# zju3dv/NeuralRecon-W

Hardware: NVIDIA H100
Metric: training rays/sec (higher is better)
Workload: dtype bf16 (3-product split forward, plain bf16 backward, fp32 accumulate)

## Files before the change

### neuralrecon-w_b200/csrc/epilogue_fast.cuh

```cuda
#pragma once
#include "epilogue_tc.cuh"

namespace nrw {

enum EpiKind {
  EK_GENERIC = 0,
  EK_FWD_SOFTPLUS,
  EK_FWD_RELU,
  EK_FWD_NONE,
  EK_GATE_FWD,
  EK_TANGENT,
  EK_REVERSE,
  EK_RELU_BWD,
  EK_FWD_HEAD,
  EK_COUNT
};

inline int pick_epi_kind(const Epi& e) {
  auto al16 = [](const void* p) { return (reinterpret_cast<uintptr_t>(p) & 15) == 0; };
  auto rows16 = [&](const void* p, int ld) { return !p || (al16(p) && (ld & 3) == 0); };
  if (e.head_w || e.head_partial)
    return (e.head_w && e.head_partial && e.bias && al16(e.bias) && al16(e.head_w) && e.act == ACT_SOFTPLUS100 && e.scale == 1.0f && e.n_planes == 0 &&
            !e.atomic && !e.aux_u.p && !e.rowvec && !e.aux_relu && !e.out_pre && !e.out2 && !e.out_f32 &&
            !e.colsum && !e.aux_add && e.n_store >= (1 << 29)) ? EK_FWD_HEAD : -1;
  if (e.atomic || e.n_planes > 3) return EK_GENERIC;
  if (e.n_planes > 0 && (!al16(e.out_pl.p) || (e.out_pl.ld & 3) || (e.out_pl.pstride & 7))) return EK_GENERIC;
  if (e.aux_u.p && (!al16(e.aux_u.p) || (e.aux_u.ld & 3) || (e.aux_u.pstride & 7))) return EK_GENERIC;
  if (!rows16(e.out_pre.p, e.out_pre.ld) || !rows16(e.out2.p, e.out2.ld) || !rows16(e.aux_add.p, e.aux_add.ld) ||
      !rows16(e.aux_q.p, e.aux_q_bcast ? 0 : e.aux_q.ld) || !rows16(e.out_f32, e.ld_f32) || !rows16(e.aux_relu, e.ld_relu) ||
      !al16(e.bias) || !al16(e.colvec))
    return EK_GENERIC;
  const bool gate = e.aux_u.p != nullptr;
  if (gate && e.out_pre && !e.out2 && !e.aux_add && !e.colsum && !e.bias && !e.rowvec && !e.aux_relu && e.n_planes > 0 && !e.out_f32)
    return EK_GATE_FWD;
  if (gate && e.out2 && e.aux_q && !e.out_pre && !e.bias && !e.rowvec && !e.aux_add && !e.colsum && !e.aux_relu &&
      ((e.n_planes > 0) != (e.out_f32 != nullptr)))
    return EK_TANGENT;
  if (gate && e.aux_add && !e.out2 && !e.out_pre && !e.bias && !e.aux_relu && e.n_planes > 0 && !e.out_f32) return EK_REVERSE;
  if (!gate && e.aux_relu && !e.out_pre && !e.out2 && !e.aux_add && !e.bias && e.n_planes > 0 && !e.out_f32 && e.act == ACT_NONE)
    return EK_RELU_BWD;
  if (!gate && e.bias && !e.rowvec && !e.aux_relu && !e.aux_add && !e.out_pre && !e.out2 && !e.out_f32 && !e.colsum && e.n_planes > 0) {
    if (e.act == ACT_SOFTPLUS100) return EK_FWD_SOFTPLUS;
    if (e.act == ACT_RELU) return EK_FWD_RELU;
    if (e.act == ACT_NONE) return EK_FWD_NONE;
  }
  return EK_GENERIC;
}

#define NRW_GATE_K (-144.269504088896341f)

template <int EK>
__device__ __forceinline__ void epi_fast16(const Epi& e, float* stg, const float (&v)[16], int m0w, int nc, int M, int N, int lane,
                                           float* cs_tile, float* hacc) {
  if constexpr (EK == EK_GENERIC) {
    epi_chunk16(e, stg, v, m0w, nc, M, N, lane, cs_tile);
  } else if constexpr (EK == EK_FWD_HEAD) {
    const int col = nc + (lane & 3) * 4;
    const float4 b = ldg4(e.bias + col), hw = ldg4(e.head_w + col);
    float x[16];
    line_transpose(stg, v, lane, x);
#pragma unroll
    for (int it = 0; it < 4; ++it) {
      float p = softplus100(x[4 * it] + b.x) * hw.x;
      p = fmaf(softplus100(x[4 * it + 1] + b.y), hw.y, p);
      p = fmaf(softplus100(x[4 * it + 2] + b.z), hw.z, p);
      p = fmaf(softplus100(x[4 * it + 3] + b.w), hw.w, p);
      p += __shfl_xor_sync(0xFFFFFFFFu, p, 1);
      p += __shfl_xor_sync(0xFFFFFFFFu, p, 2);
      hacc[it] += p;
    }
  } else {
    if (M - m0w < 32 || N - nc < 16 || e.n_store - nc < 16) {
      epi_chunk16(e, stg, v, m0w, nc, M, N, lane, cs_tile);
      return;
    }
    const int col = nc + (lane & 3) * 4;
    const long long row = (long long)m0w + (lane >> 2);
    float u[16];
    float s[16];
    float4 b;
    if constexpr (EK == EK_GATE_FWD || EK == EK_TANGENT || EK == EK_REVERSE) {
      tile_load_bf16(e.aux_u.p + row * e.aux_u.ld + col, e.aux_u.ld, u);
      if constexpr (EK == EK_GATE_FWD) {
        if (e.aux_u_planes > 1) tile_load_bf16(e.aux_u.plane(1) + row * e.aux_u.ld + col, e.aux_u.ld, s);
      }
    }
    if constexpr (EK == EK_FWD_SOFTPLUS || EK == EK_FWD_RELU || EK == EK_FWD_NONE) b = ldg4(e.bias + col);
    if constexpr (EK == EK_TANGENT) {
      if (e.aux_q_bcast) {
        const float4 qb = ldg4(e.aux_q.f32() + col);
#pragma unroll
        for (int it = 0; it < 4; ++it) { s[4 * it] = qb.x; s[4 * it + 1] = qb.y; s[4 * it + 2] = qb.z; s[4 * it + 3] = qb.w; }
      } else {
        tile_load(e.aux_q, row, col, s);
      }
    }
    if constexpr (EK == EK_REVERSE) tile_load(e.aux_add, row, col, s);
    if constexpr (EK == EK_RELU_BWD) tile_load_bf16(e.aux_relu + row * e.ld_relu + col, e.ld_relu, u);
    float x[16], w[16];
    line_transpose(stg, v, lane, x);

    if constexpr (EK == EK_FWD_SOFTPLUS || EK == EK_FWD_RELU || EK == EK_FWD_NONE) {
      const float bb[4] = {b.x, b.y, b.z, b.w};
#pragma unroll
      for (int i = 0; i < 16; ++i) {
        const float t = x[i] + bb[i & 3];
        if constexpr (EK == EK_FWD_SOFTPLUS) w[i] = softplus100(t) * e.scale;
        else if constexpr (EK == EK_FWD_RELU) w[i] = fmaxf(t, 0.0f) * e.scale;
        else w[i] = t * e.scale;
      }
    }
    if constexpr (EK == EK_REVERSE || EK == EK_RELU_BWD) {
      if (e.rowvec) {
        const float4 c = ldg4(e.colvec + col);
        const float cc[4] = {c.x, c.y, c.z, c.w};
#pragma unroll
        for (int it = 0; it < 4; ++it) {
          const float rv = __ldg(e.rowvec + row + it * 8);
#pragma unroll
          for (int k = 0; k < 4; ++k) x[4 * it + k] = fmaf(rv, cc[k], x[4 * it + k]);
        }
      }
    }
    if constexpr (EK == EK_GATE_FWD) tile_store(e.out_pre, row, col, x);
    if constexpr (EK == EK_GATE_FWD || EK == EK_TANGENT || EK == EK_REVERSE) {
      if constexpr (EK == EK_GATE_FWD) {
        if (e.aux_u_planes > 1) {
#pragma unroll
          for (int i = 0; i < 16; ++i) u[i] += s[i];
        }
      }
      for (int pl = EK == EK_GATE_FWD ? 2 : 1; pl < e.aux_u_planes; ++pl) {
        float t[16];
        tile_load_bf16(e.aux_u.plane(pl) + row * e.aux_u.ld + col, e.aux_u.ld, t);
#pragma unroll
        for (int i = 0; i < 16; ++i) u[i] += t[i];
      }
      const float kk = NRW_GATE_K * e.aux_u_scale, sc = e.scale;
      if constexpr (EK == EK_TANGENT) {
        const float sc100 = 100.0f * sc;
#pragma unroll
        for (int i = 0; i < 16; ++i) {
          const float ee = mufu_ex2(u[i] * kk);
          const float s1 = 1.0f - ee;
          const float xs = x[i] * s1;
          w[i] = xs * sc;
          s[i] = (xs * s[i]) * (ee * sc100);
        }
        tile_store(e.out2, row, col, s);
      } else if constexpr (EK == EK_REVERSE) {
#pragma unroll
        for (int i = 0; i < 16; ++i) {
          const float ee = mufu_ex2(u[i] * kk);
          w[i] = fmaf(x[i], fmaf(-sc, ee, sc), s[i]);
        }
      } else {
#pragma unroll
        for (int i = 0; i < 16; ++i) {
          const float ee = mufu_ex2(u[i] * kk);
          w[i] = x[i] * fmaf(-sc, ee, sc);
        }
      }
    }
    if constexpr (EK == EK_RELU_BWD) {
#pragma unroll
      for (int i = 0; i < 16; ++i) w[i] = u[i] > 0.0f ? x[i] * e.scale : 0.0f;
    }
    if constexpr (EK == EK_REVERSE || EK == EK_RELU_BWD) {
      if (cs_tile) line_colsum_add(w, lane, cs_tile);
    }
    if constexpr (EK == EK_TANGENT) {
      if (e.out_f32) tile_store_f32(e.out_f32 + row * e.ld_f32 + col, e.ld_f32, w);
    }
    for (int pl = 0; pl < e.n_planes; ++pl) {
      uint32_t pk[8];
      if (pl + 1 < e.n_planes) split_plane<16>(w, pk);
      else pack_bf16(w, pk);
      tile_store_bf16(e.out_pl.plane(pl) + row * e.out_pl.ld + col, e.out_pl.ld, pk);
    }
  }
}

}
```

### neuralrecon-w_b200/csrc/epilogue_tc.cuh

```cuda
#pragma once
#include "epilogue.cuh"

namespace nrw {

struct LineLayout {
  int sl;
  int r0;
  int rows_valid;
  bool full;
};

__device__ __forceinline__ bool aligned16(const void* p) { return (reinterpret_cast<uintptr_t>(p) & 15) == 0; }
__device__ __forceinline__ bool aligned8(const void* p) { return (reinterpret_cast<uintptr_t>(p) & 7) == 0; }

__device__ __forceinline__ void line_transpose(float* stg, const float (&v)[16], int lane, float (&x)[16]) {
  const int sl = lane & 3, r0 = lane >> 2;
#pragma unroll
  for (int s = 0; s < 4; ++s)
    *reinterpret_cast<float4*>(stg + lane * 16 + ((s ^ ((lane >> 1) & 3)) << 2)) = make_float4(v[4 * s], v[4 * s + 1], v[4 * s + 2], v[4 * s + 3]);
  __syncwarp();
#pragma unroll
  for (int it = 0; it < 4; ++it) {
    const int rr = it * 8 + r0;
    const float4 t = *reinterpret_cast<const float4*>(stg + rr * 16 + ((sl ^ ((rr >> 1) & 3)) << 2));
    x[4 * it] = t.x; x[4 * it + 1] = t.y; x[4 * it + 2] = t.z; x[4 * it + 3] = t.w;
  }
  __syncwarp();
}

__device__ __forceinline__ float4 ldg4(const float* p) {
  float4 v;
  asm volatile("ld.global.nc.L2::256B.v4.f32 {%0, %1, %2, %3}, [%4];" : "=f"(v.x), "=f"(v.y), "=f"(v.z), "=f"(v.w) : "l"(p));
  return v;
}
__device__ __forceinline__ uint2 ldg2u(const bf16* p) {
  uint2 v;
  asm volatile("ld.global.nc.L2::256B.v2.u32 {%0, %1}, [%2];" : "=r"(v.x), "=r"(v.y) : "l"(p));
  return v;
}

__device__ __forceinline__ void tile_load_f32(const float* p, long long ld, float (&o)[16]) {
#pragma unroll
  for (int it = 0; it < 4; ++it) {
    const float4 t = ldg4(p + it * 8 * ld);
    o[4 * it] = t.x; o[4 * it + 1] = t.y; o[4 * it + 2] = t.z; o[4 * it + 3] = t.w;
  }
}
__device__ __forceinline__ void tile_load_bf16(const bf16* p, long long ld, float (&o)[16]) {
#pragma unroll
  for (int it = 0; it < 4; ++it) {
    const uint2 t = ldg2u(p + it * 8 * ld);
    o[4 * it] = __uint_as_float(t.x << 16); o[4 * it + 1] = __uint_as_float(t.x & 0xFFFF0000u);
    o[4 * it + 2] = __uint_as_float(t.y << 16); o[4 * it + 3] = __uint_as_float(t.y & 0xFFFF0000u);
  }
}
__device__ __forceinline__ void tile_store_f32(float* p, long long ld, const float (&o)[16]) {
#pragma unroll
  for (int it = 0; it < 4; ++it)
    *reinterpret_cast<float4*>(p + it * 8 * ld) = make_float4(o[4 * it], o[4 * it + 1], o[4 * it + 2], o[4 * it + 3]);
}
__device__ __forceinline__ void tile_store_bf16(bf16* p, long long ld, const uint32_t (&pk)[8]) {
#pragma unroll
  for (int it = 0; it < 4; ++it) *reinterpret_cast<uint2*>(p + it * 8 * ld) = make_uint2(pk[2 * it], pk[2 * it + 1]);
}
__device__ __forceinline__ void pack_bf16(const float (&w)[16], uint32_t (&pk)[8]) {
#pragma unroll
  for (int t = 0; t < 8; ++t) {
    const __nv_bfloat162 h = __floats2bfloat162_rn(w[2 * t], w[2 * t + 1]);
    pk[t] = *reinterpret_cast<const uint32_t*>(&h);
  }
}
__device__ __forceinline__ void tile_load(const SideStream& s, long long row, int col, float (&o)[16]) {
  if (s.is_bf16()) tile_load_bf16(s.h() + row * s.ld + col, s.ld, o);
  else tile_load_f32(s.f32() + row * s.ld + col, s.ld, o);
}
__device__ __forceinline__ void tile_store(const SideStream& s, long long row, int col, const float (&o)[16]) {
  if (s.is_bf16()) {
    uint32_t pk[8];
    pack_bf16(o, pk);
    tile_store_bf16(s.h() + row * s.ld + col, s.ld, pk);
  } else {
    tile_store_f32(s.f32() + row * s.ld + col, s.ld, o);
  }
}

__device__ __forceinline__ bool line_fast(const LineLayout& L, const void* p, long long ld, int ncols) {
  return L.full && ncols >= 16 && aligned16(p) && (ld & 3) == 0;
}
__device__ __forceinline__ void line_load_f32(const LineLayout& L, const float* __restrict__ src, long long ld, int ncols,
                                              float (&o)[16]) {
  if (line_fast(L, src, ld, ncols)) {
    tile_load_f32(src + L.r0 * ld + L.sl * 4, ld, o);
    return;
  }
#pragma unroll
  for (int it = 0; it < 4; ++it) {
    const int rr = it * 8 + L.r0;
#pragma unroll
    for (int k = 0; k < 4; ++k) {
      const int c = L.sl * 4 + k;
      o[4 * it + k] = (rr < L.rows_valid && c < ncols) ? src[(long long)rr * ld + c] : 0.0f;
    }
  }
}
__device__ __forceinline__ void line_store_f32(const LineLayout& L, float* __restrict__ dst, long long ld, int ncols,
                                               const float (&o)[16], bool atomic) {
  if (!atomic && line_fast(L, dst, ld, ncols)) {
    tile_store_f32(dst + L.r0 * ld + L.sl * 4, ld, o);
    return;
  }
#pragma unroll
  for (int it = 0; it < 4; ++it) {
    const int rr = it * 8 + L.r0;
#pragma unroll
    for (int k = 0; k < 4; ++k) {
      const int c = L.sl * 4 + k;
      if (rr < L.rows_valid && c < ncols) {
        if (atomic) atomicAdd(dst + (long long)rr * ld + c, o[4 * it + k]);
        else dst[(long long)rr * ld + c] = o[4 * it + k];
      }
    }
  }
}
__device__ __forceinline__ void line_store_bf16(const LineLayout& L, bf16* __restrict__ dst, long long ld, int ncols,
                                                const uint32_t (&pk)[8]) {
  if (L.full && ncols >= 16 && aligned8(dst) && (ld & 3) == 0) {
    tile_store_bf16(dst + L.r0 * ld + L.sl * 4, ld, pk);
    return;
  }
#pragma unroll
  for (int it = 0; it < 4; ++it) {
    const int rr = it * 8 + L.r0;
#pragma unroll
    for (int k = 0; k < 4; ++k) {
      const int c = L.sl * 4 + k;
      if (rr < L.rows_valid && c < ncols)
        dst[(long long)rr * ld + c] = __ushort_as_bfloat16((unsigned short)((pk[2 * it + (k >> 1)] >> ((k & 1) * 16)) & 0xFFFFu));
    }
  }
}
__device__ __forceinline__ void line_load_planes(const LineLayout& L, const Planes& P, int n_planes, long long m0w, int nc, int ncols,
                                                 float scale, float (&o)[16]) {
#pragma unroll
  for (int i = 0; i < 16; ++i) o[i] = 0.0f;
  for (int pl = 0; pl < n_planes; ++pl) {
    const bf16* src = P.plane(pl) + m0w * P.ld + nc;
    if (L.full && ncols >= 16 && aligned8(src) && (P.ld & 3) == 0) {
      float t[16];
      tile_load_bf16(src + L.r0 * P.ld + L.sl * 4, P.ld, t);
#pragma unroll
      for (int i = 0; i < 16; ++i) o[i] += t[i];
    } else {
#pragma unroll
      for (int it = 0; it < 4; ++it) {
        const int rr = it * 8 + L.r0;
#pragma unroll
        for (int k = 0; k < 4; ++k) {
          const int c = L.sl * 4 + k;
          if (rr < L.rows_valid && c < ncols) o[4 * it + k] += __bfloat162float(src[(long long)rr * P.ld + c]);
        }
      }
    }
  }
  if (scale != 1.0f) {
#pragma unroll
    for (int i = 0; i < 16; ++i) o[i] *= scale;
  }
}
__device__ __forceinline__ void line_load_cols(const LineLayout& L, const float* __restrict__ vec, int ncols, float (&b)[4]) {
  const float* p = vec + L.sl * 4;
  if (ncols >= 16 && aligned16(vec)) {
    const float4 t = __ldg(reinterpret_cast<const float4*>(p));
    b[0] = t.x; b[1] = t.y; b[2] = t.z; b[3] = t.w;
  } else {
#pragma unroll
    for (int k = 0; k < 4; ++k) b[k] = (L.sl * 4 + k < ncols) ? p[k] : 0.0f;
  }
}
__device__ __forceinline__ void line_load(const LineLayout& L, const SideStream& s, long long m0w, int nc, int ncols, float (&o)[16]) {
  if (s.is_bf16()) line_load_planes(L, Planes{s.h(), 0, s.ld}, 1, m0w, nc, ncols, 1.0f, o);
  else line_load_f32(L, s.f32() + m0w * s.ld + nc, s.ld, ncols, o);
}
__device__ __forceinline__ void line_store(const LineLayout& L, const SideStream& s, long long m0w, int nc, int ncols,
                                           const float (&o)[16]) {
  if (s.is_bf16()) {
    uint32_t pk[8];
    pack_bf16(o, pk);
    line_store_bf16(L, s.h() + m0w * s.ld + nc, s.ld, ncols, pk);
  } else {
    line_store_f32(L, s.f32() + m0w * s.ld + nc, s.ld, ncols, o, false);
  }
}

__device__ __forceinline__ void line_colsum_add(const float (&w)[16], int lane, float* cs_tile) {
  float c0 = (w[0] + w[4]) + (w[8] + w[12]), c1 = (w[1] + w[5]) + (w[9] + w[13]);
  float c2 = (w[2] + w[6]) + (w[10] + w[14]), c3 = (w[3] + w[7]) + (w[11] + w[15]);
  const bool hi16 = (lane & 16) != 0, hi8 = (lane & 8) != 0;
  const float s0 = hi16 ? c0 : c2, s1 = hi16 ? c1 : c3;
  float k0 = hi16 ? c2 : c0, k1 = hi16 ? c3 : c1;
  k0 += __shfl_xor_sync(0xFFFFFFFFu, s0, 16);
  k1 += __shfl_xor_sync(0xFFFFFFFFu, s1, 16);
  const float s = hi8 ? k0 : k1;
  float k = hi8 ? k1 : k0;
  k += __shfl_xor_sync(0xFFFFFFFFu, s, 8);
  k += __shfl_xor_sync(0xFFFFFFFFu, k, 4);
  if ((lane & 4) == 0) atomicAdd(cs_tile + (lane & 3) * 4 + (hi16 ? 2 : 0) + (hi8 ? 1 : 0), k);
}

__device__ __forceinline__ void epi_chunk16(const Epi& e, float* stg, const float (&v)[16], int m0w, int nc, int M, int N, int lane,
                                            float* cs_tile) {
  LineLayout L;
  L.rows_valid = min(32, M - m0w);
  if (L.rows_valid <= 0) return;
  const int n_all = min(N - nc, 16);
  const int n_st = min(e.n_store - nc, n_all);
  L.sl = lane & 3;
  L.r0 = lane >> 2;
  L.full = L.rows_valid == 32;
  float x[16];
  line_transpose(stg, v, lane, x);
  if (e.bias) {
    float b[4];
    line_load_cols(L, e.bias + nc, n_all, b);
#pragma unroll
    for (int i = 0; i < 16; ++i) x[i] += b[i & 3];
  }
  if (e.rowvec) {
    float cv[4];
    line_load_cols(L, e.colvec + nc, n_all, cv);
#pragma unroll
    for (int it = 0; it < 4; ++it) {
      const float rv = e.rowvec[min(m0w + it * 8 + L.r0, M - 1)];
#pragma unroll
      for (int k = 0; k < 4; ++k) x[4 * it + k] = fmaf(rv, cv[k], x[4 * it + k]);
    }
  }
  if (e.out_pre) line_store(L, e.out_pre, m0w, nc, n_all, x);
  if (n_st <= 0) return;
  if (e.atomic) {
    if (e.scale != 1.0f) {
#pragma unroll
      for (int i = 0; i < 16; ++i) x[i] *= e.scale;
    }
    line_store_f32(L, e.out_f32 + (long long)m0w * e.ld_f32 + nc, e.ld_f32, n_st, x, true);
    return;
  }
  float w[16];
  if (e.aux_u.p) {
    float a[16];
    line_load_planes(L, e.aux_u, e.aux_u_planes, m0w, nc, n_st, e.aux_u_scale, a);
    if (e.out2) {
      float q[16];
      if (e.aux_q_bcast) {
        float qb[4];
        line_load_cols(L, e.aux_q.f32() + nc, n_st, qb);
#pragma unroll
        for (int i = 0; i < 16; ++i) q[i] = qb[i & 3];
      } else {
        line_load(L, e.aux_q, m0w, nc, n_st, q);
      }
#pragma unroll
      for (int i = 0; i < 16; ++i) {
        float s1, s2;
        softplus100_d12_from_u(a[i], s1, s2);
        w[i] = x[i] * s1 * e.scale;
        q[i] = e.scale * x[i] * q[i] * s2;
      }
      line_store(L, e.out2, m0w, nc, n_st, q);
    } else {
#pragma unroll
      for (int i = 0; i < 16; ++i) {
        float s1, s2;
        softplus100_d12_from_u(a[i], s1, s2);
        w[i] = x[i] * s1 * e.scale;
      }
    }
  } else {
    switch (e.act) {
      case ACT_SOFTPLUS100:
#pragma unroll
        for (int i = 0; i < 16; ++i) w[i] = softplus100(x[i]) * e.scale;
        break;
      case ACT_RELU:
#pragma unroll
        for (int i = 0; i < 16; ++i) w[i] = fmaxf(x[i], 0.0f) * e.scale;
        break;
      case ACT_SIGMOID:
#pragma unroll
        for (int i = 0; i < 16; ++i) w[i] = sigmoidf_(x[i]) * e.scale;
        break;
      default:
#pragma unroll
        for (int i = 0; i < 16; ++i) w[i] = x[i] * e.scale;
    }
    if (e.aux_relu) {
      float f[16];
      line_load_planes(L, Planes{const_cast<bf16*>(e.aux_relu), 0, e.ld_relu}, 1, m0w, nc, n_st, 1.0f, f);
#pragma unroll
      for (int i = 0; i < 16; ++i)
        if (!(f[i] > 0.0f)) w[i] = 0.0f;
    }
  }
  if (e.aux_add) {
// ... 32 lines not shown
```

### neuralrecon-w_b200/csrc/gemm_tc.cu

```cuda
#include <stdlib.h>

#include <mutex>
#include <unordered_map>
#include <vector>
#include <algorithm>
#include <stdio.h>

#include "gemm.h"
#include "epilogue_fast.cuh"

namespace nrw {

static constexpr int BM = 128;
static constexpr int BK = 64;
static constexpr int RING_BYTES = 192 * 1024;
static constexpr int MAX_STAGES = 8;
static constexpr int N_CONSUMER_WARPS = 8;
static constexpr int N_THREADS = 32 * N_CONSUMER_WARPS + 128;
static constexpr int PRODUCER_REGS = 40, CONSUMER_REGS = 232;
static constexpr int EPI_LD = 36;
static constexpr int EPI_WG_BYTES = 64 * EPI_LD * 4;
static constexpr int CS_BYTES = 1024;
static constexpr int BAR_TURN = 4;
static_assert(PRODUCER_REGS * 128 + CONSUMER_REGS * 32 * N_CONSUMER_WARPS <= 65536, "register file");
static constexpr int BAR_BYTES = 256;
static constexpr int SMEM_BYTES = 1024 + RING_BYTES + BAR_BYTES + 2 * EPI_WG_BYTES + CS_BYTES;
static_assert(SMEM_BYTES <= 232448, "dynamic shared memory limit of sm_90");
static_assert(4 * 2048 <= EPI_WG_BYTES, "the 2 KB per-warp epilogue tiles live in the warpgroup's staging tile");

struct TcParams {
  CUtensorMap tmA[3];
  CUtensorMap tmB[3];
  int M, N, K;
  int n_planes;
  int k_slices;
  int m_tiles, n_tiles;
  Epi epi;
  unsigned long long* prof;
};
#define NRW_PROF_T0(cond) const long long _t0 = (cond) ? clock64() : 0
#define NRW_PROF_ADD(cond, slot) \
  if (cond) atomicAdd(&p.prof[blockIdx.x * 16 + (slot)], (unsigned long long)(clock64() - _t0))

__device__ __forceinline__ uint32_t smem_u32(const void* p) {
  return static_cast<uint32_t>(__cvta_generic_to_shared(p));
}
__device__ __forceinline__ void mbar_init(uint32_t bar, uint32_t count) {
  asm volatile("mbarrier.init.shared::cta.b64 [%0], %1;" ::"r"(bar), "r"(count));
}
__device__ __forceinline__ void mbar_wait(uint32_t bar, uint32_t parity) {
  asm volatile(
      "{\n"
      ".reg .pred p;\n"
      "WAIT_LOOP:\n"
      "mbarrier.try_wait.parity.shared::cta.b64 p, [%0], %1;\n"
      "@p bra.uni WAIT_DONE;\n"
      "bra.uni WAIT_LOOP;\n"
      "WAIT_DONE:\n"
      "}\n" ::"r"(bar),
      "r"(parity)
      : "memory");
}
__device__ __forceinline__ void mbar_arrive(uint32_t bar) {
  asm volatile("mbarrier.arrive.shared::cta.b64 _, [%0];" ::"r"(bar) : "memory");
}
__device__ __forceinline__ void mbar_arrive_expect_tx(uint32_t bar, uint32_t bytes) {
  asm volatile("mbarrier.arrive.expect_tx.shared::cta.b64 _, [%0], %1;" ::"r"(bar), "r"(bytes)
               : "memory");
}
__device__ __forceinline__ void tma_load_2d(uint32_t dst, const CUtensorMap* map, uint32_t bar,
                                            int x, int y) {
  asm volatile(
      "cp.async.bulk.tensor.2d.shared::cluster.global.mbarrier::complete_tx::bytes"
      " [%0], [%1, {%3, %4}], [%2];" ::"r"(dst),
      "l"(reinterpret_cast<uint64_t>(map)), "r"(bar), "r"(x), "r"(y)
      : "memory");
}
__device__ __forceinline__ void tma_prefetch_desc(const CUtensorMap* map) {
  asm volatile("prefetch.tensormap [%0];" ::"l"(reinterpret_cast<uint64_t>(map)) : "memory");
}
__device__ __forceinline__ void pdl_wait() { asm volatile("griddepcontrol.wait;" ::: "memory"); }
__device__ __forceinline__ void pdl_launch_dependents() { asm volatile("griddepcontrol.launch_dependents;" ::: "memory"); }
__device__ __forceinline__ void named_bar_sync(int id, int n) { asm volatile("bar.sync %0, %1;" ::"r"(id), "r"(n) : "memory"); }
__device__ __forceinline__ void named_bar_arrive(int id, int n) { asm volatile("bar.arrive %0, %1;" ::"r"(id), "r"(n) : "memory"); }
template <int R>
__device__ __forceinline__ void setmaxnreg_inc() { asm volatile("setmaxnreg.inc.sync.aligned.u32 %0;" ::"n"(R)); }
template <int R>
__device__ __forceinline__ void setmaxnreg_dec() { asm volatile("setmaxnreg.dec.sync.aligned.u32 %0;" ::"n"(R)); }
__device__ __forceinline__ void fence_proxy_async_smem() { asm volatile("fence.proxy.async.shared::cta;" ::: "memory"); }

__device__ __forceinline__ uint64_t make_gdesc(uint32_t saddr, uint32_t lbo_bytes, uint32_t sbo_bytes) {
  uint64_t d = 0;
  d |= (uint64_t)((saddr & 0x3FFFF) >> 4);
  d |= (uint64_t)((lbo_bytes >> 4) & 0x3FFF) << 16;
  d |= (uint64_t)((sbo_bytes >> 4) & 0x3FFF) << 32;
  d |= (uint64_t)1 << 62;
  return d;
}
__device__ __forceinline__ void wgmma_fence() { asm volatile("wgmma.fence.sync.aligned;" ::: "memory"); }
__device__ __forceinline__ void wgmma_commit() { asm volatile("wgmma.commit_group.sync.aligned;" ::: "memory"); }
template <int N>
__device__ __forceinline__ void wgmma_wait() { asm volatile("wgmma.wait_group.sync.aligned %0;" ::"n"(N) : "memory"); }
template <int N>
__device__ __forceinline__ void acc_fence(float (&d)[N]) {
#pragma unroll
  for (int i = 0; i < N; ++i) asm volatile("" : "+f"(d[i])::"memory");
}

template <int BN, int TA, int TB>
__device__ __forceinline__ void wgmma_bf16(float (&d)[BN / 2], uint64_t da, uint64_t db, uint32_t accumulate);

// ... 53 lines not shown
  constexpr int B_TILE = BN * BK * 2;
  constexpr int WG_A = 64 * BK * 2;
  extern __shared__ uint8_t smem_raw[];
  uint8_t* smem = smem_raw + ((1024u - (smem_u32(smem_raw) & 1023u)) & 1023u);
  const int P = p.n_planes;
  const int stage_bytes = P * (A_TILE + B_TILE);
  int stages = RING_BYTES / stage_bytes;
  if (stages > MAX_STAGES) stages = MAX_STAGES;
  uint64_t* bars = reinterpret_cast<uint64_t*>(smem + RING_BYTES);
  const uint32_t bar_full = smem_u32(bars), bar_empty = smem_u32(bars + MAX_STAGES);
  float* epi_buf = reinterpret_cast<float*>(smem + RING_BYTES + BAR_BYTES);
  float* cs_buf = reinterpret_cast<float*>(smem + RING_BYTES + BAR_BYTES + 2 * EPI_WG_BYTES);
  const int warp = threadIdx.x >> 5, lane = threadIdx.x & 31;
  const long long t_kernel0 = clock64();

  if (warp == N_CONSUMER_WARPS && lane == 0) {
    for (int i = 0; i < P; ++i) {
      tma_prefetch_desc(&p.tmA[i]);
      tma_prefetch_desc(&p.tmB[i]);
    }
    for (int i = 0; i < MAX_STAGES; ++i) {
      mbar_init(bar_full + 8 * i, 1);
      mbar_init(bar_empty + 8 * i, 4);
    }
    asm volatile("fence.mbarrier_init.release.cluster;" ::: "memory");
  }
  if (threadIdx.x < 256) cs_buf[threadIdx.x] = 0.0f;
  __syncthreads();
  pdl_wait();
  pdl_launch_dependents();

  const int kb_total = (p.K + BK - 1) / BK;
  const int kb_per = (kb_total + p.k_slices - 1) / p.k_slices;
  const int n_items = p.m_tiles * p.n_tiles * p.k_slices;
  const int n_prod = (P == 1) ? 1 : (P == 2 ? 3 : 6);

  if (warp >= N_CONSUMER_WARPS) {
    setmaxnreg_dec<PRODUCER_REGS>();
    if (warp == N_CONSUMER_WARPS && lane == 0) {
      int s = 0;
      uint32_t ph = 0;
      for (int item = blockIdx.x; item < n_items; item += gridDim.x) {
        const int ks = item % p.k_slices;
        const int t = item / p.k_slices;
        const int n0 = (t % p.n_tiles) * BN, m0 = (t / p.n_tiles) * BM;
        const int kb0 = ks * kb_per, kb1 = min(kb_total, kb0 + kb_per);
        for (int kb = kb0; kb < kb1; ++kb) {
          {
            NRW_PROF_T0(p.prof != nullptr);
            mbar_wait(bar_empty + 8 * s, ph ^ 1);
            NRW_PROF_ADD(p.prof != nullptr, 0);
          }
          mbar_arrive_expect_tx(bar_full + 8 * s, stage_bytes);
          const uint32_t sa = smem_u32(smem + s * stage_bytes);
          const uint32_t sb = sa + P * A_TILE;
          for (int pl = 0; pl < P; ++pl) {
            if (MN_MAJOR == 0) {
              tma_load_2d(sa + pl * A_TILE, &p.tmA[pl], bar_full + 8 * s, kb * BK, m0);
              tma_load_2d(sb + pl * B_TILE, &p.tmB[pl], bar_full + 8 * s, kb * BK, n0);
            } else {
#pragma unroll
              for (int sl = 0; sl < BM / 64; ++sl)
                tma_load_2d(sa + pl * A_TILE + sl * (64 * BK * 2), &p.tmA[pl], bar_full + 8 * s,
                            m0 + 64 * sl, kb * BK);
#pragma unroll
              for (int sl = 0; sl < BN / 64; ++sl)
                tma_load_2d(sb + pl * B_TILE + sl * (64 * BK * 2), &p.tmB[pl], bar_full + 8 * s,
                            n0 + 64 * sl, kb * BK);
            }
          }
          if (++s == stages) { s = 0; ph ^= 1; }
        }
      }
    }
  } else {
    setmaxnreg_inc<CONSUMER_REGS>();
    const int wg = warp >> 2, wi = warp & 3;
    const uint32_t smem0 = smem_u32(smem);
    constexpr uint32_t LBO = MN_MAJOR ? (64 * BK * 2) : 16;
    constexpr uint32_t SBO = 1024;
    constexpr uint32_t KSTEP = MN_MAJOR ? (16 * 128) : 32;
    const uint64_t desc_hi = make_gdesc(0, LBO, SBO);
    float* stage_tile = epi_buf + wg * (EPI_WG_BYTES / 4);
    float* stg = stage_tile + wi * 512;
    const bool use_cs = p.epi.colsum != nullptr && !p.epi.atomic;
    float* cs_wg = cs_buf + 128 * wg;
    const int ctid = threadIdx.x & 127;
    const bool prof = p.prof != nullptr && wi == 0 && lane == 0;
    const int po = 8 * wg;
    int cs_n0 = -1;
    int s = 0;
    uint32_t ph = 0;
    for (int j = 0; blockIdx.x + j * gridDim.x < n_items; ++j) {
      const int item = blockIdx.x + j * gridDim.x;
      const int ks = item % p.k_slices;
      const int t = item / p.k_slices;
      const int n0 = (t % p.n_tiles) * BN, m0 = (t / p.n_tiles) * BM;
      const int kb0 = ks * kb_per, kb1 = min(kb_total, kb0 + kb_per);
      if ((j & 1) != wg) {
        for (int kb = kb0; kb < kb1; ++kb)
          if (++s == stages) { s = 0; ph ^= 1; }
        continue;
      }
      if (use_cs && n0 != cs_n0) {
        if (cs_n0 >= 0) colsum_flush(cs_wg, p.epi.colsum, cs_n0, min(min(p.N, p.epi.n_store) - cs_n0, BN), ctid, 128, 2 + wg);
        cs_n0 = n0;
      }
      float acc[2][BN / 2];
#pragma unroll
      for (int h = 0; h < 2; ++h)
#pragma unroll
        for (int i = 0; i < BN / 2; ++i) acc[h][i] = 0.0f;
      if (j > 0) {
        NRW_PROF_T0(prof);
        named_bar_sync(BAR_TURN + wg, 256);
        NRW_PROF_ADD(prof, 3 + po);
      }
      int prev_s = -1;
      for (int kb = kb0; kb < kb1; ++kb) {
        {
          NRW_PROF_T0(prof);
          mbar_wait(bar_full + 8 * s, ph);
          NRW_PROF_ADD(prof, 1 + po);
        }
        const uint32_t sa = smem0 + s * stage_bytes;
        const uint32_t sb = smem0 + s * stage_bytes + P * A_TILE;
        wgmma_fence();
        for (int pr = 0; pr < n_prod; ++pr) {
          const int q = 4 * (n_prod - 1 - pr);
          const uint32_t pa = (0x021010u >> q) & 0xFu, pb = (0x201100u >> q) & 0xFu;
          const uint64_t da = desc_hi | (uint64_t)(((sa + pa * A_TILE) & 0x3FFFFu) >> 4);
          const uint64_t db = desc_hi | (uint64_t)(((sb + pb * B_TILE) & 0x3FFFFu) >> 4);
#pragma unroll
          for (int k = 0; k < BK / 16; ++k)
#pragma unroll
            for (int h = 0; h < 2; ++h)
              wgmma_bf16<BN, MN_MAJOR, MN_MAJOR>(acc[h], da + ((h * WG_A + k * KSTEP) >> 4), db + ((k * KSTEP) >> 4), 1u);
        }
        wgmma_commit();
        acc_fence(acc[0]);
        acc_fence(acc[1]);
        if (prev_s >= 0) {
          wgmma_wait<1>();
          acc_fence(acc[0]);
          acc_fence(acc[1]);
          if (lane == 0) mbar_arrive(bar_empty + 8 * prev_s);
        }
        prev_s = s;
        if (++s == stages) { s = 0; ph ^= 1; }
      }
      if (item + gridDim.x < n_items) named_bar_arrive(BAR_TURN + (wg ^ 1), 256);
      wgmma_wait<0>();
      acc_fence(acc[0]);
      acc_fence(acc[1]);
      if (prev_s >= 0 && lane == 0) mbar_arrive(bar_empty + 8 * prev_s);
      if (kb1 <= kb0) continue;
      NRW_PROF_T0(prof);
      if (prof) atomicAdd(&p.prof[blockIdx.x * 16 + 6 + po], 1ull);
      const int r0 = 16 * wi + (lane >> 2), c0 = 2 * (lane & 3);
      const int qq = wi & 1, cc = wi >> 1;
      const int n_cp = (min(BN, p.N - n0) + 31) / 32;
#pragma unroll
      for (int h = 0; h < 2; ++h) {
        const int m0w = m0 + 64 * h + 32 * qq;
        float hacc[4] = {0.0f, 0.0f, 0.0f, 0.0f};
#pragma unroll
        for (int cp = 0; cp < BN / 32; ++cp) {
          if (cp >= n_cp) break;
#pragma unroll
          for (int jj = 0; jj < 4; ++jj) {
            const int jf = 4 * cp + jj;
            *reinterpret_cast<float2*>(stage_tile + r0 * EPI_LD + 8 * jj + c0) = make_float2(acc[h][4 * jf], acc[h][4 * jf + 1]);
            *reinterpret_cast<float2*>(stage_tile + (r0 + 8) * EPI_LD + 8 * jj + c0) = make_float2(acc[h][4 * jf + 2], acc[h][4 * jf + 3]);
          }
          named_bar_sync(2 + wg, 128);
          float v[16];
          const float* src = stage_tile + (32 * qq + lane) * EPI_LD + 16 * cc;
#pragma unroll
          for (int i = 0; i < 4; ++i) {
            const float4 t4 = *reinterpret_cast<const float4*>(src + 4 * i);
            v[4 * i] = t4.x; v[4 * i + 1] = t4.y; v[4 * i + 2] = t4.z; v[4 * i + 3] = t4.w;
          }
          named_bar_sync(2 + wg, 128);
          const int nc = n0 + 32 * cp + 16 * cc;
          if (nc < p.N && m0w < p.M)
            epi_fast16<EK>(p.epi, stg, v, m0w, nc, p.M, p.N, lane, use_cs ? cs_wg + 32 * cp + 16 * cc : nullptr, hacc);
          named_bar_sync(2 + wg, 128);
        }
        if (EK == EK_FWD_HEAD && (lane & 3) == 0) {
          const int slot = (n0 / BN) * 2 + cc;
#pragma unroll
          for (int it = 0; it < 4; ++it) {
            const int row = m0w + it * 8 + (lane >> 2);
            if (row < p.M) p.epi.head_partial[(long long)row * 8 + slot] = hacc[it];
          }
        }
      }
      NRW_PROF_ADD(prof, 4 + po);
    }
    if (use_cs && cs_n0 >= 0) colsum_flush(cs_wg, p.epi.colsum, cs_n0, min(min(p.N, p.epi.n_store) - cs_n0, BN), ctid, 128, 2 + wg);
  }
  __syncthreads();
  if (p.prof && threadIdx.x == 0) atomicAdd(&p.prof[blockIdx.x * 16 + 5], (unsigned long long)(clock64() - t_kernel0));
}

typedef CUresult (*EncodeTiledFn)(CUtensorMap*, CUtensorMapDataType, cuuint32_t, void*, const cuuint64_t*,
                                  const cuuint64_t*, const cuuint32_t*, const cuuint32_t*,
                                  CUtensorMapInterleave, CUtensorMapSwizzle, CUtensorMapL2promotion,
                                  CUtensorMapFloatOOBfill);

static EncodeTiledFn get_encode() {
  static EncodeTiledFn fn = nullptr;
  static std::once_flag once;
  std::call_once(once, [] {
    void* sym = nullptr;
    cudaDriverEntryPointQueryResult qres;
    if (cudaGetDriverEntryPoint("cuTensorMapEncodeTiled", &sym, cudaEnableDefault, &qres) == cudaSuccess &&
        qres == cudaDriverEntryPointSuccess)
      fn = reinterpret_cast<EncodeTiledFn>(sym);
  });
  return fn;
}

struct MapKey {
  const void* ptr; long long inner, outer, ld; int box_inner, box_outer;
  bool operator==(const MapKey& o) const {
    return ptr == o.ptr && inner == o.inner && outer == o.outer && ld == o.ld &&
           box_inner == o.box_inner && box_outer == o.box_outer;
  }
};
struct MapKeyHash {
  size_t operator()(const MapKey& k) const {
    size_t h = std::hash<const void*>()(k.ptr);
    h = h * 1000003u ^ (size_t)k.inner; h = h * 1000003u ^ (size_t)k.outer;
    h = h * 1000003u ^ (size_t)k.ld; h = h * 1000003u ^ (size_t)(k.box_inner * 1024 + k.box_outer);
    return h;
  }
};
static std::unordered_map<MapKey, CUtensorMap, MapKeyHash> g_map_cache;
static std::mutex g_map_mutex;

static int make_map(CUtensorMap* out, const bf16* ptr, long long inner, long long outer, long long ld,
                    int box_inner, int box_outer, bool swizzle = true) {
  MapKey key{ptr, inner, outer, ld, swizzle ? box_inner : -box_inner, box_outer};
  {
    std::lock_guard<std::mutex> lk(g_map_mutex);
    auto it = g_map_cache.find(key);
    if (it != g_map_cache.end()) { *out = it->second; return NRW_OK; }
  }
  EncodeTiledFn enc = get_encode();
  NRW_CHECK(enc != nullptr, NRW_ERR_CUDA, "cuTensorMapEncodeTiled entry point unavailable");
  NRW_CHECK((reinterpret_cast<uintptr_t>(ptr) & 15) == 0 && (ld % 8) == 0, NRW_ERR_ARG,
            "TMA operand must be 16B aligned with ld %% 8 == 0 (ptr=%p ld=%lld)", (const void*)ptr, ld);
  cuuint64_t dims[2] = {(cuuint64_t)inner, (cuuint64_t)outer};
  cuuint64_t strides[1] = {(cuuint64_t)ld * 2};
  cuuint32_t box[2] = {(cuuint32_t)box_inner, (cuuint32_t)box_outer};
  cuuint32_t estr[2] = {1, 1};
  CUresult r = enc(out, CU_TENSOR_MAP_DATA_TYPE_BFLOAT16, 2, const_cast<bf16*>(ptr), dims, strides, box, estr,
                   CU_TENSOR_MAP_INTERLEAVE_NONE, swizzle ? CU_TENSOR_MAP_SWIZZLE_128B : CU_TENSOR_MAP_SWIZZLE_NONE,
                   CU_TENSOR_MAP_L2_PROMOTION_L2_256B, CU_TENSOR_MAP_FLOAT_OOB_FILL_NONE);
  NRW_CHECK(r == CUDA_SUCCESS, NRW_ERR_CUDA, "cuTensorMapEncodeTiled failed (%d) inner=%lld outer=%lld ld=%lld",
            (int)r, inner, outer, ld);
  std::lock_guard<std::mutex> lk(g_map_mutex);
  if (g_map_cache.size() > 65536) g_map_cache.clear();
  g_map_cache.emplace(key, *out);
  return NRW_OK;
}

static unsigned long long* g_prof_ptr = nullptr;
// ... 398 lines not shown
```

Baseline: 34580.

## Stage epilogue in 64-column swizzled rounds and prefetch side inputs before barrier

Reworks the GEMM epilogue so each warpgroup stages 64 accumulator columns per round into a swizzled shared-memory tile. Each thread then reads its line-ordered 16-value fragments directly, which removes the separate per-warp line_transpose pass and one named barrier per chunk. For simple kinds (bias+activation, relu backward), side inputs such as bias and bf16 relu masks for both 32-column halves are loaded as raw registers before the barrier, so their global latency overlaps the staging sync. This raises register pressure from holding two FastSide structs and changes the shared-memory layout, which risks bank conflicts or spills.

```diff
diff --git a/neuralrecon-w_b200/csrc/epilogue_fast.cuh b/neuralrecon-w_b200/csrc/epilogue_fast.cuh
--- a/neuralrecon-w_b200/csrc/epilogue_fast.cuh
+++ b/neuralrecon-w_b200/csrc/epilogue_fast.cuh
@@ -49,16 +49,137 @@
 
 #define NRW_GATE_K (-144.269504088896341f)
 
-template <int EK>
-__device__ __forceinline__ void epi_fast16(const Epi& e, float* stg, const float (&v)[16], int m0w, int nc, int M, int N, int lane,
-                                           float* cs_tile, float* hacc) {
+struct FastSide {
+  uint2 u[4];
+  uint2 u2[4];
+  float s[16];
+  float4 b;
+};
+
+template <int EK>
+__device__ __forceinline__ void fast_side_load(const Epi& e, long long row, int col, FastSide& f) {
+  if constexpr (EK == EK_GATE_FWD || EK == EK_TANGENT || EK == EK_REVERSE) {
+    tile_load_bf16_raw(e.aux_u.p + row * e.aux_u.ld + col, e.aux_u.ld, f.u);
+    if constexpr (EK == EK_GATE_FWD) {
+      if (e.aux_u_planes > 1) tile_load_bf16_raw(e.aux_u.plane(1) + row * e.aux_u.ld + col, e.aux_u.ld, f.u2);
+    }
+  }
+  if constexpr (EK == EK_FWD_SOFTPLUS || EK == EK_FWD_RELU || EK == EK_FWD_NONE) f.b = ldg4(e.bias + col);
+  if constexpr (EK == EK_TANGENT) {
+    if (e.aux_q_bcast) {
+      const float4 qb = ldg4(e.aux_q.f32() + col);
+#pragma unroll
+      for (int it = 0; it < 4; ++it) { f.s[4 * it] = qb.x; f.s[4 * it + 1] = qb.y; f.s[4 * it + 2] = qb.z; f.s[4 * it + 3] = qb.w; }
+    } else {
+      tile_load(e.aux_q, row, col, f.s);
+    }
+  }
+  if constexpr (EK == EK_REVERSE) tile_load(e.aux_add, row, col, f.s);
+  if constexpr (EK == EK_RELU_BWD) tile_load_bf16_raw(e.aux_relu + row * e.ld_relu + col, e.ld_relu, f.u);
+}
+
+template <int EK>
+__device__ __forceinline__ void fast_finish(const Epi& e, const float (&x_acc)[16], long long row, int col, int lane, float* cs_tile,
+                                            const FastSide& f) {
+  float x[16], w[16];
+#pragma unroll
+  for (int i = 0; i < 16; ++i) x[i] = x_acc[i];
+  if constexpr (EK == EK_FWD_SOFTPLUS || EK == EK_FWD_RELU || EK == EK_FWD_NONE) {
+    const float bb[4] = {f.b.x, f.b.y, f.b.z, f.b.w};
+#pragma unroll
+    for (int i = 0; i < 16; ++i) {
+      const float t = x[i] + bb[i & 3];
+      if constexpr (EK == EK_FWD_SOFTPLUS) w[i] = softplus100(t) * e.scale;
+      else if constexpr (EK == EK_FWD_RELU) w[i] = fmaxf(t, 0.0f) * e.scale;
+      else w[i] = t * e.scale;
+    }
+  }
+  if constexpr (EK == EK_REVERSE || EK == EK_RELU_BWD) {
+    if (e.rowvec) {
+      const float4 c = ldg4(e.colvec + col);
+      const float cc[4] = {c.x, c.y, c.z, c.w};
+#pragma unroll
+      for (int it = 0; it < 4; ++it) {
+        const float rv = __ldg(e.rowvec + row + it * 8);
+#pragma unroll
+        for (int k = 0; k < 4; ++k) x[4 * it + k] = fmaf(rv, cc[k], x[4 * it + k]);
+      }
+    }
+  }
+  if constexpr (EK == EK_GATE_FWD) tile_store(e.out_pre, row, col, x);
+  if constexpr (EK == EK_GATE_FWD || EK == EK_TANGENT || EK == EK_REVERSE) {
+    float u[16], s[16];
+    unpack_bf16(f.u, u);
+    if constexpr (EK == EK_GATE_FWD) {
+      if (e.aux_u_planes > 1) {
+        float u2[16];
+        unpack_bf16(f.u2, u2);
+#pragma unroll
+        for (int i = 0; i < 16; ++i) u[i] += u2[i];
+      }
+    }
+    for (int pl = EK == EK_GATE_FWD ? 2 : 1; pl < e.aux_u_planes; ++pl) {
+      float t[16];
+      tile_load_bf16(e.aux_u.plane(pl) + row * e.aux_u.ld + col, e.aux_u.ld, t);
+#pragma unroll
+      for (int i = 0; i < 16; ++i) u[i] += t[i];
+    }
+#pragma unroll
+    for (int i = 0; i < 16; ++i) s[i] = f.s[i];
+    const float kk = NRW_GATE_K * e.aux_u_scale, sc = e.scale;
+    if constexpr (EK == EK_TANGENT) {
+      const float sc100 = 100.0f * sc;
+#pragma unroll
+      for (int i = 0; i < 16; ++i) {
+        const float ee = mufu_ex2(u[i] * kk);
+        const float s1 = 1.0f - ee;
+        const float xs = x[i] * s1;
+        w[i] = xs * sc;
+        s[i] = (xs * s[i]) * (ee * sc100);
+      }
+      tile_store(e.out2, row, col, s);
+    } else if constexpr (EK == EK_REVERSE) {
+#pragma unroll
+      for (int i = 0; i < 16; ++i) {
+        const float ee = mufu_ex2(u[i] * kk);
+        w[i] = fmaf(x[i], fmaf(-sc, ee, sc), s[i]);
+      }
+    } else {
+#pragma unroll
+      for (int i = 0; i < 16; ++i) {
+        const float ee = mufu_ex2(u[i] * kk);
+        w[i] = x[i] * fmaf(-sc, ee, sc);
+      }
+    }
+  }
+  if constexpr (EK == EK_RELU_BWD) {
+    float fw[16];
+    unpack_bf16(f.u, fw);
+#pragma unroll
+    for (int i = 0; i < 16; ++i) w[i] = fw[i] > 0.0f ? x[i] * e.scale : 0.0f;
+  }
+  if constexpr (EK == EK_REVERSE || EK == EK_RELU_BWD) {
+    if (cs_tile) line_colsum_add(w, lane, cs_tile);
+  }
+  if constexpr (EK == EK_TANGENT) {
+    if (e.out_f32) tile_store_f32(e.out_f32 + row * e.ld_f32 + col, e.ld_f32, w);
+  }
+  for (int pl = 0; pl < e.n_planes; ++pl) {
+    uint32_t pk[8];
+    if (pl + 1 < e.n_planes) split_plane<16>(w, pk);
+    else pack_bf16(w, pk);
+    tile_store_bf16(e.out_pl.plane(pl) + row * e.out_pl.ld + col, e.out_pl.ld, pk);
+  }
+}
+
+template <int EK>
+__device__ __forceinline__ void epi_fast16(const Epi& e, const float (&x)[16], int m0w, int nc, int M, int N, int lane, float* cs_tile,
+                                           float* hacc) {
   if constexpr (EK == EK_GENERIC) {
-    epi_chunk16(e, stg, v, m0w, nc, M, N, lane, cs_tile);
+    epi_chunk16(e, x, m0w, nc, M, N, lane, cs_tile);
   } else if constexpr (EK == EK_FWD_HEAD) {
     const int col = nc + (lane & 3) * 4;
     const float4 b = ldg4(e.bias + col), hw = ldg4(e.head_w + col);
-    float x[16];
-    line_transpose(stg, v, lane, x);
 #pragma unroll
     for (int it = 0; it < 4; ++it) {
       float p = softplus100(x[4 * it] + b.x) * hw.x;
@@ -71,114 +192,43 @@
     }
   } else {
     if (M - m0w < 32 || N - nc < 16 || e.n_store - nc < 16) {
-      epi_chunk16(e, stg, v, m0w, nc, M, N, lane, cs_tile);
+      epi_chunk16(e, x, m0w, nc, M, N, lane, cs_tile);
       return;
     }
     const int col = nc + (lane & 3) * 4;
     const long long row = (long long)m0w + (lane >> 2);
-    float u[16];
-    float s[16];
-    float4 b;
-    if constexpr (EK == EK_GATE_FWD || EK == EK_TANGENT || EK == EK_REVERSE) {
-      tile_load_bf16(e.aux_u.p + row * e.aux_u.ld + col, e.aux_u.ld, u);
-      if constexpr (EK == EK_GATE_FWD) {
-        if (e.aux_u_planes > 1) tile_load_bf16(e.aux_u.plane(1) + row * e.aux_u.ld + col, e.aux_u.ld, s);
-      }
-    }
-    if constexpr (EK == EK_FWD_SOFTPLUS || EK == EK_FWD_RELU || EK == EK_FWD_NONE) b = ldg4(e.bias + col);
-    if constexpr (EK == EK_TANGENT) {
-      if (e.aux_q_bcast) {
-        const float4 qb = ldg4(e.aux_q.f32() + col);
-#pragma unroll
-        for (int it = 0; it < 4; ++it) { s[4 * it] = qb.x; s[4 * it + 1] = qb.y; s[4 * it + 2] = qb.z; s[4 * it + 3] = qb.w; }
-      } else {
-        tile_load(e.aux_q, row, col, s);
-      }
-    }
-    if constexpr (EK == EK_REVERSE) tile_load(e.aux_add, row, col, s);
-    if constexpr (EK == EK_RELU_BWD) tile_load_bf16(e.aux_relu + row * e.ld_relu + col, e.ld_relu, u);
-    float x[16], w[16];
-    line_transpose(stg, v, lane, x);
-
-    if constexpr (EK == EK_FWD_SOFTPLUS || EK == EK_FWD_RELU || EK == EK_FWD_NONE) {
-      const float bb[4] = {b.x, b.y, b.z, b.w};
-#pragma unroll
-      for (int i = 0; i < 16; ++i) {
-        const float t = x[i] + bb[i & 3];
-        if constexpr (EK == EK_FWD_SOFTPLUS) w[i] = softplus100(t) * e.scale;
-        else if constexpr (EK == EK_FWD_RELU) w[i] = fmaxf(t, 0.0f) * e.scale;
-        else w[i] = t * e.scale;
-      }
-    }
-    if constexpr (EK == EK_REVERSE || EK == EK_RELU_BWD) {
-      if (e.rowvec) {
-        const float4 c = ldg4(e.colvec + col);
-        const float cc[4] = {c.x, c.y, c.z, c.w};
-#pragma unroll
-        for (int it = 0; it < 4; ++it) {
-          const float rv = __ldg(e.rowvec + row + it * 8);
-#pragma unroll
-          for (int k = 0; k < 4; ++k) x[4 * it + k] = fmaf(rv, cc[k], x[4 * it + k]);
-        }
-      }
-    }
-    if constexpr (EK == EK_GATE_FWD) tile_store(e.out_pre, row, col, x);
-    if constexpr (EK == EK_GATE_FWD || EK == EK_TANGENT || EK == EK_REVERSE) {
-      if constexpr (EK == EK_GATE_FWD) {
-        if (e.aux_u_planes > 1) {
-#pragma unroll
-          for (int i = 0; i < 16; ++i) u[i] += s[i];
-        }
-      }
-      for (int pl = EK == EK_GATE_FWD ? 2 : 1; pl < e.aux_u_planes; ++pl) {
-        float t[16];
-        tile_load_bf16(e.aux_u.plane(pl) + row * e.aux_u.ld + col, e.aux_u.ld, t);
-#pragma unroll
-        for (int i = 0; i < 16; ++i) u[i] += t[i];
-      }
-      const float kk = NRW_GATE_K * e.aux_u_scale, sc = e.scale;
-      if constexpr (EK == EK_TANGENT) {
-        const float sc100 = 100.0f * sc;
-#pragma unroll
-        for (int i = 0; i < 16; ++i) {
-          const float ee = mufu_ex2(u[i] * kk);
-          const float s1 = 1.0f - ee;
-          const float xs = x[i] * s1;
-          w[i] = xs * sc;
-          s[i] = (xs * s[i]) * (ee * sc100);
-        }
-        tile_store(e.out2, row, col, s);
-      } else if constexpr (EK == EK_REVERSE) {
-#pragma unroll
-        for (int i = 0; i < 16; ++i) {
-          const float ee = mufu_ex2(u[i] * kk);
-          w[i] = fmaf(x[i], fmaf(-sc, ee, sc), s[i]);
-        }
-      } else {
-#pragma unroll
-        for (int i = 0; i < 16; ++i) {
-          const float ee = mufu_ex2(u[i] * kk);
-          w[i] = x[i] * fmaf(-sc, ee, sc);
-        }
-      }
-    }
-    if constexpr (EK == EK_RELU_BWD) {
-#pragma unroll
-      for (int i = 0; i < 16; ++i) w[i] = u[i] > 0.0f ? x[i] * e.scale : 0.0f;
-    }
-    if constexpr (EK == EK_REVERSE || EK == EK_RELU_BWD) {
-      if (cs_tile) line_colsum_add(w, lane, cs_tile);
-    }
-    if constexpr (EK == EK_TANGENT) {
-      if (e.out_f32) tile_store_f32(e.out_f32 + row * e.ld_f32 + col, e.ld_f32, w);
-    }
-    for (int pl = 0; pl < e.n_planes; ++pl) {
-      uint32_t pk[8];
-      if (pl + 1 < e.n_planes) split_plane<16>(w, pk);
-      else pack_bf16(w, pk);
-      tile_store_bf16(e.out_pl.plane(pl) + row * e.out_pl.ld + col, e.out_pl.ld, pk);
-    }
-  }
-}
-
-}
+    FastSide f;
+    fast_side_load<EK>(e, row, col, f);
+    fast_finish<EK>(e, x, row, col, lane, cs_tile, f);
+  }
+}
+
+template <int EK>
+constexpr bool pair_kind() {
+  return EK == EK_FWD_SOFTPLUS || EK == EK_FWD_RELU || EK == EK_FWD_NONE || EK == EK_RELU_BWD;
+}
+template <int EK>
+__device__ __forceinline__ bool pair_full(const Epi& e, int m0w, int nc, int M, int N) {
+  if constexpr (!pair_kind<EK>()) return false;
+  else return M - m0w >= 32 && N - (nc + 32) >= 16 && e.n_store - (nc + 32) >= 16;
+}
+template <int EK>
+__device__ __forceinline__ void pair_load(const Epi& e, int m0w, int nc, int lane, FastSide& f0, FastSide& f1) {
+  const int col = nc + (lane & 3) * 4;
+  const long long row = (long long)m0w + (lane >> 2);
+  fast_side_load<EK>(e, row, col, f0);
+  fast_side_load<EK>(e, row, col + 32, f1);
+}
+template <int EK>
+__device__ __forceinline__ void epi_pair_chunk(const Epi& e, const float (&x)[16], bool full, const FastSide& f, int m0w, int nc, int M,
+                                               int N, int lane, float* cs_tile, float* hacc) {
+  if constexpr (pair_kind<EK>()) {
+    if (full) {
+      fast_finish<EK>(e, x, (long long)m0w + (lane >> 2), nc + (lane & 3) * 4, lane, cs_tile, f);
+      return;
+    }
+  }
+  epi_fast16<EK>(e, x, m0w, nc, M, N, lane, cs_tile, hacc);
+}
+
+}
diff --git a/neuralrecon-w_b200/csrc/epilogue_tc.cuh b/neuralrecon-w_b200/csrc/epilogue_tc.cuh
--- a/neuralrecon-w_b200/csrc/epilogue_tc.cuh
+++ b/neuralrecon-w_b200/csrc/epilogue_tc.cuh
@@ -13,21 +13,6 @@
 __device__ __forceinline__ bool aligned16(const void* p) { return (reinterpret_cast<uintptr_t>(p) & 15) == 0; }
 __device__ __forceinline__ bool aligned8(const void* p) { return (reinterpret_cast<uintptr_t>(p) & 7) == 0; }
 
-__device__ __forceinline__ void line_transpose(float* stg, const float (&v)[16], int lane, float (&x)[16]) {
-  const int sl = lane & 3, r0 = lane >> 2;
-#pragma unroll
-  for (int s = 0; s < 4; ++s)
-    *reinterpret_cast<float4*>(stg + lane * 16 + ((s ^ ((lane >> 1) & 3)) << 2)) = make_float4(v[4 * s], v[4 * s + 1], v[4 * s + 2], v[4 * s + 3]);
-  __syncwarp();
-#pragma unroll
-  for (int it = 0; it < 4; ++it) {
-    const int rr = it * 8 + r0;
-    const float4 t = *reinterpret_cast<const float4*>(stg + rr * 16 + ((sl ^ ((rr >> 1) & 3)) << 2));
-    x[4 * it] = t.x; x[4 * it + 1] = t.y; x[4 * it + 2] = t.z; x[4 * it + 3] = t.w;
-  }
-  __syncwarp();
-}
-
 __device__ __forceinline__ float4 ldg4(const float* p) {
   float4 v;
   asm volatile("ld.global.nc.L2::256B.v4.f32 {%0, %1, %2, %3}, [%4];" : "=f"(v.x), "=f"(v.y), "=f"(v.z), "=f"(v.w) : "l"(p));
@@ -46,13 +31,22 @@
     o[4 * it] = t.x; o[4 * it + 1] = t.y; o[4 * it + 2] = t.z; o[4 * it + 3] = t.w;
   }
 }
-__device__ __forceinline__ void tile_load_bf16(const bf16* p, long long ld, float (&o)[16]) {
-#pragma unroll
-  for (int it = 0; it < 4; ++it) {
-    const uint2 t = ldg2u(p + it * 8 * ld);
+__device__ __forceinline__ void tile_load_bf16_raw(const bf16* p, long long ld, uint2 (&r)[4]) {
+#pragma unroll
+  for (int it = 0; it < 4; ++it) r[it] = ldg2u(p + it * 8 * ld);
+}
+__device__ __forceinline__ void unpack_bf16(const uint2 (&r)[4], float (&o)[16]) {
+#pragma unroll
+  for (int it = 0; it < 4; ++it) {
+    const uint2 t = r[it];
     o[4 * it] = __uint_as_float(t.x << 16); o[4 * it + 1] = __uint_as_float(t.x & 0xFFFF0000u);
     o[4 * it + 2] = __uint_as_float(t.y << 16); o[4 * it + 3] = __uint_as_float(t.y & 0xFFFF0000u);
   }
+}
+__device__ __forceinline__ void tile_load_bf16(const bf16* p, long long ld, float (&o)[16]) {
+  uint2 r[4];
+  tile_load_bf16_raw(p, ld, r);
+  unpack_bf16(r, o);
 }
 __device__ __forceinline__ void tile_store_f32(float* p, long long ld, const float (&o)[16]) {
 #pragma unroll
@@ -207,7 +201,7 @@
   if ((lane & 4) == 0) atomicAdd(cs_tile + (lane & 3) * 4 + (hi16 ? 2 : 0) + (hi8 ? 1 : 0), k);
 }
 
-__device__ __forceinline__ void epi_chunk16(const Epi& e, float* stg, const float (&v)[16], int m0w, int nc, int M, int N, int lane,
+__device__ __forceinline__ void epi_chunk16(const Epi& e, const float (&x_acc)[16], int m0w, int nc, int M, int N, int lane,
                                             float* cs_tile) {
   LineLayout L;
   L.rows_valid = min(32, M - m0w);
@@ -218,7 +212,8 @@
   L.r0 = lane >> 2;
   L.full = L.rows_valid == 32;
   float x[16];
-  line_transpose(stg, v, lane, x);
+#pragma unroll
+  for (int i = 0; i < 16; ++i) x[i] = x_acc[i];
   if (e.bias) {
     float b[4];
     line_load_cols(L, e.bias + nc, n_all, b);
diff --git a/neuralrecon-w_b200/csrc/gemm_tc.cu b/neuralrecon-w_b200/csrc/gemm_tc.cu
--- a/neuralrecon-w_b200/csrc/gemm_tc.cu
+++ b/neuralrecon-w_b200/csrc/gemm_tc.cu
@@ -18,15 +18,16 @@
 static constexpr int N_CONSUMER_WARPS = 8;
 static constexpr int N_THREADS = 32 * N_CONSUMER_WARPS + 128;
 static constexpr int PRODUCER_REGS = 40, CONSUMER_REGS = 232;
-static constexpr int EPI_LD = 36;
-static constexpr int EPI_WG_BYTES = 64 * EPI_LD * 4;
+static constexpr int EPI_COLS = 64;
+static constexpr int EPI_WG_BYTES = 64 * EPI_COLS * 4;
 static constexpr int CS_BYTES = 1024;
 static constexpr int BAR_TURN = 4;
 static_assert(PRODUCER_REGS * 128 + CONSUMER_REGS * 32 * N_CONSUMER_WARPS <= 65536, "register file");
 static constexpr int BAR_BYTES = 256;
 static constexpr int SMEM_BYTES = 1024 + RING_BYTES + BAR_BYTES + 2 * EPI_WG_BYTES + CS_BYTES;
 static_assert(SMEM_BYTES <= 232448, "dynamic shared memory limit of sm_90");
-static_assert(4 * 2048 <= EPI_WG_BYTES, "the 2 KB per-warp epilogue tiles live in the warpgroup's staging tile");
+
+__device__ __forceinline__ int epi_swz(int r) { return ((r & 1) << 2) | (r & 2) | ((r >> 2) & 1); }
 
 struct TcParams {
   CUtensorMap tmA[3];
@@ -246,7 +247,6 @@
     constexpr uint32_t KSTEP = MN_MAJOR ? (16 * 128) : 32;
     const uint64_t desc_hi = make_gdesc(0, LBO, SBO);
     float* stage_tile = epi_buf + wg * (EPI_WG_BYTES / 4);
-    float* stg = stage_tile + wi * 512;
     const bool use_cs = p.epi.colsum != nullptr && !p.epi.atomic;
     float* cs_wg = cs_buf + 128 * wg;
     const int ctid = threadIdx.x & 127;
@@ -323,32 +323,45 @@
       if (prof) atomicAdd(&p.prof[blockIdx.x * 16 + 6 + po], 1ull);
       const int r0 = 16 * wi + (lane >> 2), c0 = 2 * (lane & 3);
       const int qq = wi & 1, cc = wi >> 1;
-      const int n_cp = (min(BN, p.N - n0) + 31) / 32;
+      const int n_rounds = (min(BN, p.N - n0) + EPI_COLS - 1) / EPI_COLS;
+      float* st_w = stage_tile + r0 * EPI_COLS + (c0 & 3);
+      const int st_x = (c0 >> 2) ^ epi_swz(r0);
+      const float* st_l = stage_tile + (32 * qq + (lane >> 2)) * EPI_COLS;
+      const int ln_x = (lane & 3) ^ epi_swz(lane >> 2);
 #pragma unroll
       for (int h = 0; h < 2; ++h) {
         const int m0w = m0 + 64 * h + 32 * qq;
         float hacc[4] = {0.0f, 0.0f, 0.0f, 0.0f};
 #pragma unroll
-        for (int cp = 0; cp < BN / 32; ++cp) {
-          if (cp >= n_cp) break;
-#pragma unroll
-          for (int jj = 0; jj < 4; ++jj) {
-            const int jf = 4 * cp + jj;
-            *reinterpret_cast<float2*>(stage_tile + r0 * EPI_LD + 8 * jj + c0) = make_float2(acc[h][4 * jf], acc[h][4 * jf + 1]);
-            *reinterpret_cast<float2*>(stage_tile + (r0 + 8) * EPI_LD + 8 * jj + c0) = make_float2(acc[h][4 * jf + 2], acc[h][4 * jf + 3]);
-          }
+        for (int rd = 0; rd < BN / EPI_COLS; ++rd) {
+          if (rd >= n_rounds) break;
+          const int nc = n0 + EPI_COLS * rd + 16 * cc;
+          const bool act = nc < p.N && m0w < p.M;
+          const bool full = act && pair_full<EK>(p.epi, m0w, nc, p.M, p.N);
+#pragma unroll
+          for (int jj = 0; jj < 8; ++jj) {
+            const int jf = 8 * rd + jj;
+            float* d = st_w + (((2 * jj) ^ st_x) << 2);
+            *reinterpret_cast<float2*>(d) = make_float2(acc[h][4 * jf], acc[h][4 * jf + 1]);
+            *reinterpret_cast<float2*>(d + 8 * EPI_COLS) = make_float2(acc[h][4 * jf + 2], acc[h][4 * jf + 3]);
+          }
+          FastSide f0, f1;
+          if (full) pair_load<EK>(p.epi, m0w, nc, lane, f0, f1);
           named_bar_sync(2 + wg, 128);
-          float v[16];
-          const float* src = stage_tile + (32 * qq + lane) * EPI_LD + 16 * cc;
-#pragma unroll
-          for (int i = 0; i < 4; ++i) {
-            const float4 t4 = *reinterpret_cast<const float4*>(src + 4 * i);
-            v[4 * i] = t4.x; v[4 * i + 1] = t4.y; v[4 * i + 2] = t4.z; v[4 * i + 3] = t4.w;
-          }
-          named_bar_sync(2 + wg, 128);
-          const int nc = n0 + 32 * cp + 16 * cc;
-          if (nc < p.N && m0w < p.M)
-            epi_fast16<EK>(p.epi, stg, v, m0w, nc, p.M, p.N, lane, use_cs ? cs_wg + 32 * cp + 16 * cc : nullptr, hacc);
+          if (act) {
+            float* cs = use_cs ? cs_wg + EPI_COLS * rd + 16 * cc : nullptr;
+#pragma unroll
+            for (int c = 0; c < 2; ++c) {
+              if (c == 1 && nc + 32 >= p.N) break;
+              float x[16];
+#pragma unroll
+              for (int it = 0; it < 4; ++it) {
+                const float4 t = *reinterpret_cast<const float4*>(st_l + it * 8 * EPI_COLS + (((4 * cc + 8 * c) ^ ln_x) << 2));
+                x[4 * it] = t.x; x[4 * it + 1] = t.y; x[4 * it + 2] = t.z; x[4 * it + 3] = t.w;
+              }
+              epi_pair_chunk<EK>(p.epi, x, full, c ? f1 : f0, m0w, nc + 32 * c, p.M, p.N, lane, cs ? cs + 32 * c : nullptr, hacc);
+            }
+          }
           named_bar_sync(2 + wg, 128);
         }
         if (EK == EK_FWD_HEAD && (lane & 3) == 0) {
```

New measurement: 36550 (median of 6 runs). +5.7%, better.
